# TangJiakai/RecBole-FairRec

Hardware: AMD Instinct MI355X
Metric: training interactions/sec + achieved HBM GB/s, FOCF emb=64 at 1/2/4/8 MI355X (higher is better)
Workload: dtype f32; 1 GPU; FOCF fair_objective=value, 1000001 users x 100001 items, embedding_size=64, B=8192 per GPU, Adam lr=1e-3 weight_decay=1e-3 (BASELINE.json configs[1]); ranks_seen=1, item_distribution=uniform, launch=hipGraph, lazy_adam_sweep_period=123, tables=single GPU, global_batch=8192, aged_steps=123

## Files before the change

### include/fairrec_hip.h

```cpp
#ifndef FAIRREC_HIP_H
#define FAIRREC_HIP_H

#include <stddef.h>
#include <stdint.h>

#ifdef __cplusplus
extern "C" {
#endif

#if defined(__GNUC__) || defined(__clang__)
#define FR_API __attribute__((visibility("default")))
#else
#define FR_API
#endif

#define FR_OK 0
#define FR_EINVAL (-1)
#define FR_EHIP (-2)
#define FR_EUNSUPPORTED (-3)

#define FR_DEV_ERR_INDEX_RANGE 1u
#define FR_DEV_ERR_SST_GROUPS 2u

#define FR_DEV_ERR_BUCKET_OVERFLOW 4u
// ... 57 lines not shown
    const float* sst;
    int64_t B;
    void* ws;
    size_t ws_bytes;
    const float* rating;
} fr_focf_batch;
FR_API int fr_focf_prepare_many(const fr_focf_batch* batches, int32_t n, int64_t n_users, int64_t n_items, int32_t dim,
                         uint32_t* err_flag, void* stream);

FR_API int fr_focf_clip_grad_norm(const fr_table* U, const fr_table* I, int64_t B, float max_norm,
                           const float* extra_sqnorm, float* norm_out, void* ws, size_t ws_bytes, void* stream);

FR_API int fr_focf_backward_adam(const fr_table* U, const fr_table* I, const fr_adam* adam, int64_t B,
                          int32_t sweep_period, void* ws, size_t ws_bytes, void* stream);

FR_API int fr_focf_prepare_step(const fr_focf_batch* batches, const int32_t* stamps, int32_t n, const fr_table* U,
                                const fr_table* I, int32_t replay_cap, uint32_t* err_flag, void* stream);
FR_API int fr_focf_step(const fr_table* U, const fr_table* I, const fr_adam* adam, const int64_t* user,
                        const int64_t* item, const float* rating, const float* sst, int64_t B, int32_t objective,
                        float fair_weight, int32_t sweep_period, int32_t stamp, void* ws, size_t ws_bytes,
                        float* loss_out, void* prev_ws, int64_t prev_B, float* prev_loss_out, float* loss_acc,
                        uint32_t* err_flag, void* stream);
FR_API int fr_focf_step_finish(void* ws, size_t ws_bytes, int64_t B, int32_t dim, int32_t objective, float fair_weight,
                               float* loss_out, float* loss_acc, void* stream);
FR_API int fr_focf_step_runs(const fr_table* U, const fr_table* I, const fr_adam* adam, const int64_t* user,
                             const int64_t* item, const float* rating, const float* sst, int64_t B, int32_t objective,
                             float fair_weight, int32_t sweep_period, int32_t stamp, void* ws, size_t ws_bytes, void* prev_ws,
                             int64_t prev_B, float* prev_loss_out, float* loss_acc, uint32_t* err_flag, void* stream);
FR_API int fr_focf_step_runs_pipe(const fr_table* U, const fr_table* I, const fr_adam* adam, const int64_t* user,
                                  const int64_t* item, const float* rating, const float* sst, int64_t B, int32_t objective,
                                  float fair_weight, int32_t sweep_period, int32_t stamp, void* ws, size_t ws_bytes, void* fin_ws,
                                  int64_t fin_B, int32_t fin_step, void* prev_ws, int64_t prev_B, float* prev_loss_out,
                                  float* loss_acc, int32_t* own_u, int32_t* own_i, uint32_t* err_flag, void* stream);

FR_API size_t fr_focf_row_words(int64_t n_users, int64_t n_items);
FR_API int fr_focf_stage(const fr_table* U, const fr_table* I, const fr_focf_batch* claim, int32_t claim_stamp,
                         int32_t claim_gen, const fr_focf_batch* place, int32_t place_stamp, int32_t place_gen,
                         int32_t sweep_period, uint64_t* row_words, uint32_t* err_flag, void* stream);
FR_API int fr_focf_step_staged(const fr_table* U, const fr_table* I, const fr_adam* adam, const float* sst, int64_t B,
                               int32_t objective, float fair_weight, int32_t sweep_period, int32_t stamp, int32_t gen,
                               void* ws, size_t ws_bytes, void* prev_ws, int64_t prev_B, float* prev_loss_out,
                               float* loss_acc, uint64_t* row_words, const fr_focf_batch* claim, int32_t claim_stamp,
                               int32_t claim_gen, const fr_focf_batch* place, int32_t place_stamp, int32_t place_gen,
                               uint32_t* err_flag, void* stream);
FR_API int fr_focf_step_finish_staged(void* ws, size_t ws_bytes, int64_t B, int32_t dim, int32_t objective,
                                      float fair_weight, float* loss_out, float* loss_acc, void* stream);
FR_API int fr_focf_runs_many(const fr_table* U, const fr_table* I, const fr_adam* adam, const fr_focf_batch* batches,
                             int32_t n, int32_t objective, float fair_weight, int32_t sweep_period, int32_t first_stamp,
                             void* fin_ws, int64_t fin_B, int32_t fin_step, float* fin_loss_out, void* prev_ws, int64_t prev_B,
                             float* prev_loss_out, float* loss_ring, int32_t loss_slots, int32_t first_slot, float* loss_acc,
                             int32_t* own_u, int32_t* own_i, uint32_t* err_flag, void* stream);
FR_API int fr_focf_steps_many(const fr_table* U, const fr_table* I, const fr_adam* adam, const fr_focf_batch* batches,
                              int32_t n, int32_t objective, float fair_weight, int32_t sweep_period, int32_t first_stamp,
                              int32_t first_gen, void* prev_ws, int64_t prev_B, float* prev_loss_out, float* loss_ring,
                              int32_t loss_slots, int32_t first_slot, float* loss_acc, uint64_t* row_words,
                              uint32_t* err_flag, void* stream);

FR_API int fr_focf_predict(const fr_table* U, const fr_table* I, const fr_adam* adam, const int64_t* user,
                    const int64_t* item, int64_t B, float max_rating, float* out, uint32_t* err_flag, void* stream);


FR_API int fr_table_flush(const fr_table* t, const fr_adam* adam, void* stream);

FR_API int fr_table_gather(const fr_table* t, const fr_adam* adam, const int64_t* idx, int64_t M, float* out,
                    uint32_t* err_flag, void* stream);

// ... 435 lines not shown
```

### recbole-fairrec_amd/csrc/focf_gather.hpp

```cpp
#pragma once
#include "common.hpp"
#include "kernels.hpp"
#include "table.hpp"
#include "focf_ws.hpp"

namespace fr {

template <int E, int NWAVES = GATHER_THREADS / WAVE>
struct GatherLds {
    float red[NWAVES];
    float irow[NWAVES][3][64 * E + 1];
};

struct SortedPark {
    const int32_t* pos_of;
    const int4* info;
    const float* sst;
    int4* recs;
    int4* vals;
    float* mse_e;
};

struct PipeWait {
    const int32_t *own_prev_u, *own_prev_i;
    int32_t *own_cur_u, *own_cur_i;
    int fin_step;
};

template <int E>
__device__ __forceinline__ int pipe_take_row(const TableV& T, int row, int need, RowFrag<E>& p, RowFrag<E>& m, RowFrag<E>& v,
                                             int lane, uint32_t* err) {
    int l = 0;
    for (int spin = 0; spin < (1 << 18); ++spin) {
        l = __hip_atomic_load(T.last + row, __ATOMIC_RELAXED, __HIP_MEMORY_SCOPE_AGENT);
        if (l >= need) break;
        __builtin_amdgcn_s_sleep(8);
    }
    l = uniform(l);
    if (l < need && lane == 0 && err) atomicOr(err, FR_DEV_ERR_PIPE_WAIT);
    const int D = T.D;
#pragma unroll
    for (int e = 0; e < E; ++e) {
        const int d = lane + 64 * e;
        const size_t o = (size_t)row * D + d;
        p.x[e] = d < D ? __hip_atomic_load(T.p + o, __ATOMIC_RELAXED, __HIP_MEMORY_SCOPE_AGENT) : 0.f;
        m.x[e] = d < D ? __hip_atomic_load(T.m + o, __ATOMIC_RELAXED, __HIP_MEMORY_SCOPE_AGENT) : 0.f;
        v.x[e] = d < D ? __hip_atomic_load(T.v + o, __ATOMIC_RELAXED, __HIP_MEMORY_SCOPE_AGENT) : 0.f;
    }
    return l;
}

template <int E, bool TRAIN, bool SHARE, bool SORTED = false, bool PIPE = false, int NW = GATHER_THREADS / WAVE>
__device__ __forceinline__ void focf_gather_body(
    const TableV& U, const TableV& I, const AdamC& c, const int64_t* __restrict__ user, const int64_t* __restrict__ item,
    const float* __restrict__ rating, int B, int upto_u, int upto_i, const FocfWs& w, float max_rating,
    float* __restrict__ predict_out, uint32_t* err, int block, GatherLds<SHARE ? E : 0, NW>& lds, SortedPark sp = SortedPark{},
    PipeWait pw = PipeWait{}) {
    static_assert(NW % 4 == 0, "squared errors are reduced four waves at a time");
    const int lane = threadIdx.x & 63;
    const int wib = threadIdx.x >> 6;
    const int b = block * NW + wib;
    const bool valid = b < B;
    const int D = U.D;
    float e2 = 0.f;
    int ur = 0, ir = -1 - wib;
    int js = b;
    int4 inf = make_int4(0, 0, 0, 0);
    float sv = 0.f;
    if (SORTED && valid) {
        js = sp.pos_of[b];
        inf = sp.info[b];
        if (sp.sst) sv = sp.sst[b];
    }
    if (valid) {
        long long ul = user[b], il = item[b];
        if (ul < 0 || ul >= U.n_rows || il < 0 || il >= I.n_rows) {
            if (lane == 0 && err) atomicOr(err, FR_DEV_ERR_INDEX_RANGE);
            ul = ul < 0 || ul >= U.n_rows ? 0 : ul;
            il = il < 0 || il >= I.n_rows ? 0 : il;
        }
        ur = uniform((int)ul);
        ir = uniform((int)il);
    }
    int lead = wib;
    bool shares = false;
    if (SHARE) {
        int it[NW];
#pragma unroll
        for (int q = 0; q < NW; ++q) {
            const int bq = block * NW + q;
            long long v = bq < B ? item[bq] : -1;
            it[q] = (v < 0 || v >= I.n_rows) ? (bq < B ? 0 : -1 - q) : (int)v;
        }
#pragma unroll
        for (int q = NW - 1; q >= 0; --q) {
            if (q < wib && it[q] == ir) lead = q;
#pragma unroll
            for (int r = 0; r < q; ++r) shares |= it[q] == it[r];
        }
    }
    lead = uniform(lead);
    shares = uniform((int)shares) != 0;
    RowFrag<E> pu, mu, vu, pi, mi, vi;
    if (valid) {
        int lu = U.last[ur];
        int li = lead == wib ? I.last[ir] : 0;
        int ou = -1, oi = -1;
        if (PIPE) {
            ou = pw.own_prev_u[ur];
            if (lead == wib) oi = pw.own_prev_i[ir];
        }
        load_row<E>(pu, U.p + (size_t)ur * D, D, lane);
        if (lead == wib) load_row<E>(pi, I.p + (size_t)ir * D, D, lane);
        load_row<E>(mu, U.m + (size_t)ur * D, D, lane);
        load_row<E>(vu, U.v + (size_t)ur * D, D, lane);
        if (lead == wib) {
            load_row<E>(mi, I.m + (size_t)ir * D, D, lane);
            load_row<E>(vi, I.v + (size_t)ir * D, D, lane);
        }
        if (PIPE) {
            if (pw.fin_step >= 0 && uniform(ou) == pw.fin_step) lu = pipe_take_row<E>(U, ur, pw.fin_step, pu, mu, vu, lane, err);
            if (lead == wib && pw.fin_step >= 0 && uniform(oi) == pw.fin_step)
                li = pipe_take_row<E>(I, ir, pw.fin_step, pi, mi, vi, lane, err);
            if (lane == 0) {
                pw.own_cur_u[ur] = upto_u + 1;
                if (lead == wib) pw.own_cur_i[ir] = upto_i + 1;
            }
        }
#ifdef FR_DIAG_GATHER_NO_REPLAY
        if (PIPE) lu = upto_u, li = upto_i;
#endif
        const int t0u = uniform(lu);
        if (lead != wib) {
            replay<E>(pu, mu, vu, t0u, upto_u, c, lane);
        } else {
            const int t0i = uniform(li);
            if (upto_u == upto_i) {
                if (t0u < t0i) replay<E>(pu, mu, vu, t0u, t0i, c, lane);
                else if (t0i < t0u) replay<E>(pi, mi, vi, t0i, t0u, c, lane);
                replay2<E>(pu, mu, vu, pi, mi, vi, t0u > t0i ? t0u : t0i, upto_u, c, lane);
            } else {
                replay<E>(pu, mu, vu, t0u, upto_u, c, lane);
                replay<E>(pi, mi, vi, t0i, upto_i, c, lane);
            }
        }
    }
    if (SHARE && shares) {
        if (valid && lead == wib) {
#pragma unroll
            for (int e = 0; e < E; ++e) {
                lds.irow[wib][0][lane + 64 * e] = pi.x[e];
                lds.irow[wib][1][lane + 64 * e] = mi.x[e];
// ... 260 lines not shown
```

### recbole-fairrec_amd/csrc/focf_runs.hip

```cpp
#include <stddef.h>
#include <stdlib.h>

#include <algorithm>
#include <vector>

#include "common.hpp"
#include "kernels.hpp"
#include "table.hpp"
#include "focf_ws.hpp"
#include "focf_loss.hpp"
#include "focf_gather.hpp"

namespace fr {

#ifndef FR_RUN_WAVES
#define FR_RUN_WAVES 8
#endif
constexpr int RUN_WAVES = FR_RUN_WAVES;
constexpr int RUN_THREADS = 64 * RUN_WAVES;
#ifndef FR_RUN_DIAG
#define FR_RUN_DIAG 0
#endif
#ifndef FR_RUN_MB1
#define FR_RUN_MB1 8
// ... 376 lines not shown
    blk -= 1;
    if (blk >= a.n_item_blocks) {
        const long long wave = (long long)(blk - a.n_item_blocks) * RUN_WAVES + wv;
        if (wave < a.n_sweep_waves) sweep_slice_wave<E>(a.U, a.I, a.c, a.sw, a.sweep_wave0 + wave, lane);
        return;
    }
    for (int k = blk; k < a.B; k += a.n_item_blocks) {
        const int rK = G(a.w.nseg_i)[0], rj0 = G(a.w.seg_start_i)[k], rj1 = G(a.w.seg_start_i)[k + 1];
        const int rir = G(a.w.seg_row_i)[k];
        if (k >= uniform(rK) || FR_RUN_DIAG == 4) break;
        const int j0 = uniform(rj0);
        run_finish_item<E>(a, k, j0, uniform(rj1) - j0, uniform(rir), lds_rows, coef_s, sh, lane, wv);
        __syncthreads();
    }
}

#ifndef FR_PIPE_MB
#define FR_PIPE_MB 4
#endif
struct PipeArgs {
    RunArgs fin;
    TableV U, I;
    AdamC c;
    const int64_t *user, *item;
    const float* rating;
    int B, upto;
    FocfWs w;
    SortedPark sp;
    PipeWait pw;
    uint32_t* err;
    int n_fin_blocks, n_gather_blocks, n_sweep_blocks, n_sweep_front;
    SweepSlice sw;
    long long n_sweep_waves;
};

#ifndef FR_PIPE_PRIO
#define FR_PIPE_PRIO 1
#endif
#ifndef FR_PIPE_WPE
#define FR_PIPE_WPE 8
#endif
#ifndef FR_PIPE_PAIR_MAX_E
#define FR_PIPE_PAIR_MAX_E 0
#endif
__host__ __device__ constexpr bool pipe_pair(int E) { return E <= FR_PIPE_PAIR_MAX_E; }
#ifdef FR_PIPE_TRACE
__device__ unsigned long long pipe_dbg[8 * 8];
struct PipeSpan {
    int role, slot;
    __device__ PipeSpan(int r, int step) : role(r), slot(step & 7) {
        if (r == 0 && threadIdx.x < 8) pipe_dbg[((step + 4) & 7) * 8 + threadIdx.x] = (threadIdx.x & 1) ? 0ull : ~0ull;
        if (threadIdx.x == 0 && (blockIdx.x & 15) == 0) atomicMin(&pipe_dbg[slot * 8 + 2 * role], __builtin_amdgcn_s_memrealtime());
    }
    __device__ ~PipeSpan() {
        if ((threadIdx.x & 63) == 0 && (blockIdx.x & 15) == 0) atomicMax(&pipe_dbg[slot * 8 + 2 * role + 1], __builtin_amdgcn_s_memrealtime());
    }
};
#define PIPE_SPAN(r) PipeSpan span_(r, p.upto)
#else
#define PIPE_SPAN(r) do {} while (0)
#endif

template <int E>
__global__ __launch_bounds__(RUN_THREADS) __attribute__((amdgpu_waves_per_eu(FR_PIPE_WPE, FR_PIPE_WPE))) void focf_runs_pipe_kernel(PipeArgs p) {
    constexpr int CAP = run_cap(E);
    __shared__ __align__(16) float lds_rows[CAP * 64 * E];
    __shared__ float coef_s[CAP];
    __shared__ float sh[4];
    using GLds = GatherLds<E, pipe_pair(E) ? 2 * RUN_WAVES : RUN_WAVES>;
    static_assert(sizeof(GLds) <= sizeof(lds_rows), "the gather's LDS fits the item runs' row buffer");
    GLds& glds = *reinterpret_cast<GLds*>(lds_rows);
    const int lane = threadIdx.x & 63, wv = threadIdx.x >> 6;
    int blk = (int)blockIdx.x;
    if (blk == 0) {
        PIPE_SPAN(0);
        const RunArgs a = args_through_vgprs<RunArgs>(lane);
        if (a.prev.loss_out && threadIdx.x < 256) step_reduce_loss<256>(a.prev);
        return;
    }
    blk -= 1;
    if (blk < p.n_sweep_front) {
        PIPE_SPAN(1);
        const long long wave = (long long)blk * RUN_WAVES + wv;
        if (wave < p.n_sweep_waves) sweep_slice_wave<E>(p.U, p.I, p.c, p.sw, wave, lane);
        return;
    }
    blk -= p.n_sweep_front;
    if (blk < p.n_fin_blocks) {
        PIPE_SPAN(2);
#if FR_PIPE_PRIO
        __builtin_amdgcn_s_setprio(3);
#endif
        const RunArgs a = args_through_vgprs<RunArgs>(lane);
        for (int k = blk; k < a.B; k += a.n_item_blocks) {
            const int rK = G(a.w.nseg_i)[0], rj0 = G(a.w.seg_start_i)[k], rj1 = G(a.w.seg_start_i)[k + 1];
            const int rir = G(a.w.seg_row_i)[k];
            if (k >= uniform(rK)) break;
            const int j0 = uniform(rj0);
            run_finish_item<E, FR_PIPE_MB>(a, k, j0, uniform(rj1) - j0, uniform(rir), lds_rows, coef_s, sh, lane, wv);
            __syncthreads();
        }
        return;
    }
    blk -= p.n_fin_blocks;
    if (blk < p.n_gather_blocks) {
        PIPE_SPAN(3);
#if FR_PIPE_PRIO
        __builtin_amdgcn_s_setprio(2);
#endif
        if (blk == 0 && threadIdx.x == 0) *p.w.defer = DeferLoss{nullptr, 0, 0.f, 0};
        if constexpr (pipe_pair(E))
            focf_gather_pair_body<E, RUN_WAVES>(p.U, p.I, p.c, p.user, p.item, p.rating, p.B, p.upto, p.w, p.err, blk, glds, p.sp, p.pw);
        else
            focf_gather_body<E, true, true, true, true, RUN_WAVES>(p.U, p.I, p.c, p.user, p.item, p.rating, p.B, p.upto, p.upto, p.w,
                                                                   0.f, nullptr, p.err, blk, glds, p.sp, p.pw);
        return;
    }
    blk -= p.n_gather_blocks;
    {
        PIPE_SPAN(1);
        const long long wave = (long long)(p.n_sweep_front + blk) * RUN_WAVES + wv;
        if (wave < p.n_sweep_waves) sweep_slice_wave<E>(p.U, p.I, p.c, p.sw, wave, lane);
    }
}

}

using namespace fr;

#ifdef FR_PIPE_TRACE
extern "C" __attribute__((visibility("default"))) int fr_debug_pipe_trace(unsigned long long* out, int reset) {
    if (hipMemcpyFromSymbol(out, HIP_SYMBOL(pipe_dbg), sizeof(unsigned long long) * 64) != hipSuccess) return -1;
    if (reset) {
        unsigned long long init[64];
        for (int i = 0; i < 64; ++i) init[i] = (i & 1) ? 0ull : ~0ull;
        if (hipMemcpyToSymbol(HIP_SYMBOL(pipe_dbg), init, sizeof(init)) != hipSuccess) return -1;
    }
    return 0;
}
#endif

extern "C" int fr_focf_step_runs_pipe(const fr_table* U, const fr_table* I, const fr_adam* adam, const int64_t* user,
                                      const int64_t* item, const float* rating, const float* sst, int64_t B, int32_t objective,
                                      float fair_weight, int32_t sweep_period, int32_t stamp, void* ws, size_t ws_bytes,
                                      void* fin_ws, int64_t fin_B, int32_t fin_step, void* prev_ws, int64_t prev_B,
                                      float* prev_loss_out, float* loss_acc, int32_t* own_u, int32_t* own_i, uint32_t* err_flag,
                                      void* stream_) {
    hipStream_t stream = (hipStream_t)stream_;
    int rc;
    if ((rc = check_table(U, "fr_focf_step_runs_pipe(U)")) || (rc = check_table(I, "fr_focf_step_runs_pipe(I)")) ||
        (rc = check_focf_adam(adam, "fr_focf_step_runs_pipe")))
        return rc;
    const bool gather = user != nullptr && B > 0, finish = fin_ws != nullptr && fin_B > 0;
    FR_CHECK_ARG(U->dim == I->dim && U->step >= 1 && U->step == I->step && !U->step_dev && !I->step_dev,
                 "fr_focf_step_runs_pipe: tables of one width at one host-side step");
    FR_CHECK_ARG(objective >= FR_FOCF_NONE && objective <= FR_FOCF_OVER, "fr_focf_step_runs_pipe: objective %d", objective);
    FR_CHECK_ARG(!gather || (item && rating && ws && own_u && own_i && B <= FR_SORT_MAX && (objective == FR_FOCF_NONE || sst)),
                 "fr_focf_step_runs_pipe: bad batch");
    FR_CHECK_ARG(!finish || (fin_step >= 1 && fin_B <= FR_SORT_MAX && (!gather || fin_step == U->step - 1)),
                 "fr_focf_step_runs_pipe: the batch to finish must be the previous step's");
    PipeArgs p{};
    p.c = make_adamc(adam);
    p.err = err_flag;
    RunArgs& a = p.fin;
    a.c = p.c;
    a.objective = objective;
    a.fair_weight = fair_weight;
    a.err = err_flag;
    a.publish = gather ? 1 : 0;
    fr_table Uf = *U, If = *I;
    if (finish) {
        Uf.step = If.step = fin_step;
        a.w = focf_layout(fin_ws, fin_B, U->dim);
        a.B = (int)fin_B;
        a.n_item_blocks = (int)std::min<long long>(FR_RUN_ITEM_BLOCKS, fin_B);
    }
    a.U = view(&Uf);
    a.I = view(&If);
    a.prev = prev_of(prev_ws, prev_B, U->dim, objective, fair_weight, prev_loss_out, loss_acc, false);
    p.n_fin_blocks = a.n_item_blocks;
    if (gather) {
        p.w = focf_layout(ws, B, U->dim);
        FR_CHECK_ARG(ws_bytes >= p.w.bytes, "fr_focf_step_runs_pipe: workspace %zu < %zu bytes", ws_bytes, p.w.bytes);
        p.U = view(U);
        p.I = view(I);
        p.user = user;
        p.item = item;
        p.rating = rating;
        p.B = (int)B;
        p.upto = U->step - 1;
        p.sp = SortedPark{p.w.pos_i, p.w.info, sst, p.w.task_rec, p.w.task_info, p.w.mse_e};
        const int cur = U->step & 1, prv = cur ^ 1;
        p.pw = PipeWait{own_u + (size_t)prv * U->n_rows, own_i + (size_t)prv * I->n_rows, own_u + (size_t)cur * U->n_rows,
                        own_i + (size_t)cur * I->n_rows, finish ? fin_step : -1};
        const int per_block = pipe_pair((U->dim + 63) / 64) ? 2 * RUN_WAVES : RUN_WAVES;
        p.n_gather_blocks = (int)((B + per_block - 1) / per_block);
        if (sweep_period > 0) {
            p.sw = make_sweep_slice(U, I, sweep_period);
            p.sw.skip_from = finish ? std::min(stamp, fin_step) : stamp;
            p.n_sweep_waves = sweep_slice_waves(p.sw);
        }
    }
    p.n_sweep_blocks = (int)((p.n_sweep_waves + RUN_WAVES - 1) / RUN_WAVES);
    static const int front_pct = getenv("FAIRREC_PIPE_SWEEP_FRONT") ? atoi(getenv("FAIRREC_PIPE_SWEEP_FRONT")) : 100;
    p.n_sweep_front = (int)((long long)p.n_sweep_blocks * std::min(std::max(front_pct, 0), 100) / 100);
    const long long blocks = 1 + p.n_sweep_blocks + p.n_fin_blocks + p.n_gather_blocks;
    ProfScope prof(K_FOCF_STEP, stream);
    FR_DISPATCH_E(U->dim, FR_LAUNCH(prof, (focf_runs_pipe_kernel<E>), dim3((unsigned)blocks), dim3(RUN_THREADS), 0, stream, p));
    FR_CHECK_LAUNCH();
    return FR_OK;
}

extern "C" int fr_focf_step_runs(const fr_table* U, const fr_table* I, const fr_adam* adam, const int64_t* user,
                                 const int64_t* item, const float* rating, const float* sst, int64_t B, int32_t objective,
                                 float fair_weight, int32_t sweep_period, int32_t stamp, void* ws, size_t ws_bytes, void* prev_ws,
                                 int64_t prev_B, float* prev_loss_out, float* loss_acc, uint32_t* err_flag, void* stream_) {
    hipStream_t stream = (hipStream_t)stream_;
    int rc;
    if ((rc = check_table(U, "fr_focf_step_runs(U)")) || (rc = check_table(I, "fr_focf_step_runs(I)")) ||
        (rc = check_focf_adam(adam, "fr_focf_step_runs")))
        return rc;
    FR_CHECK_ARG(U->dim == I->dim, "fr_focf_step_runs: user dim %d != item dim %d", U->dim, I->dim);
    FR_CHECK_ARG(ws && user && item && rating, "fr_focf_step_runs: null pointer");
    FR_CHECK_ARG(objective >= FR_FOCF_NONE && objective <= FR_FOCF_OVER,
                 "fr_focf_step_runs: objective %d needs batch-wide statistics before the update (use fr_focf_forward)", objective);
    FR_CHECK_ARG(objective == FR_FOCF_NONE || sst, "fr_focf_step_runs: sst column required for a fairness objective");
    FR_CHECK_ARG(B >= 1 && B <= FR_SORT_MAX, "fr_focf_step_runs: batch size %lld not in 1..%d", (long long)B, FR_SORT_MAX);
    FR_CHECK_ARG(U->step >= 1 && U->step == I->step, "fr_focf_step_runs: table.step must be the step being applied (>=1), "
                 "the same for both tables");
    FR_CHECK_ARG(!U->step_dev && !I->step_dev, "fr_focf_step_runs: device step counters are not supported");
    RunArgs a{};
    a.w = focf_layout(ws, B, U->dim);
    FR_CHECK_ARG(ws_bytes >= a.w.bytes, "fr_focf_step_runs: workspace %zu < %zu bytes", ws_bytes, a.w.bytes);
    a.U = view(U);
    a.I = view(I);
    a.c = make_adamc(adam);
    a.B = (int)B;
    a.objective = objective;
    a.fair_weight = fair_weight;
    a.err = err_flag;
    static const int split_pct = getenv("FAIRREC_RUNS_SWEEP_SPLIT") ? atoi(getenv("FAIRREC_RUNS_SWEEP_SPLIT")) : 0;
    long long sweep_blocks = 0, in_gather = 0;
    if (sweep_period > 0) {
// ... 50 lines not shown
            if (done[1]) (void)hipEventDestroy(done[1]);
        }
    } ev;
    if (ss && n > G) {
        FR_CHECK_HIP(hipEventCreateWithFlags(&ev.fork, hipEventDisableTiming));
        FR_CHECK_HIP(hipEventCreateWithFlags(&ev.done[0], hipEventDisableTiming));
        FR_CHECK_HIP(hipEventCreateWithFlags(&ev.done[1], hipEventDisableTiming));
    }
    hipEvent_t ev_fork = ev.fork;
    hipEvent_t* ev_done = ev.done;
    int rc;
    auto prepare = [&](int g, hipStream_t st) {
        const int lo = g * G, cnt = std::min(G, n - lo);
        return fr_focf_prepare_step(batches + lo, stamps.data() + lo, cnt, U, I, sweep_period, err_flag, st);
    };
    if ((rc = prepare(0, stream))) return rc;
    fr_table tu = *U, ti = *I;
    for (int k = 0; k < n; ++k) {
        if (k % G == 0) {
            const int g = k / G;
            if (g > 0 && ss) FR_CHECK_HIP(hipStreamWaitEvent(stream, ev_done[g & 1], 0));
            if ((g + 1) * G < n) {
                if (ss) {
                    FR_CHECK_HIP(hipEventRecord(ev_fork, stream));
                    FR_CHECK_HIP(hipStreamWaitEvent(ss->stream, ev_fork, 0));
                    if ((rc = prepare(g + 1, ss->stream))) return rc;
                    FR_CHECK_HIP(hipEventRecord(ev_done[(g + 1) & 1], ss->stream));
                } else if ((rc = prepare(g + 1, stream))) {
                    return rc;
                }
            }
        }
        const fr_focf_batch& b = batches[k];
        rc = fr_focf_step_runs_pipe(&tu, &ti, adam, b.user, b.item, b.rating, b.sst, b.B, objective, fair_weight, sweep_period,
                                    stamps[(size_t)k], b.ws, b.ws_bytes, fin_ws, fin_B, fin_step, prev_ws, prev_B, prev_loss_out,
                                    loss_acc, own_u, own_i, err_flag, stream_);
        if (rc) return rc;
        prev_ws = fin_ws; prev_B = fin_B; prev_loss_out = fin_loss_out;
        fin_ws = b.ws; fin_B = b.B; fin_step = tu.step;
        fin_loss_out = loss_ring + 4 * (size_t)((first_slot + k) % loss_slots);
        ++tu.step; ++ti.step;
    }
    return FR_OK;
}
```

### recbole-fairrec_amd/fairrec/_C.py

```python
from __future__ import annotations

import ctypes
import os
from ctypes import POINTER, Structure, c_char_p, c_double, c_float, c_int, c_int32, c_int64, c_size_t, c_uint32, c_uint64, c_void_p

LIB_PATH = os.environ.get("FAIRREC_HIP_LIB") or os.path.join(os.path.dirname(os.path.abspath(__file__)), "lib",
                                                             "libfairrec_hip.so")

FR_SORT_MAX = 16384
DEV_ERR_INDEX_RANGE = 1
DEV_ERR_SST_GROUPS = 2
DEV_ERR_BUCKET_OVERFLOW = 4
DEV_ERR_PIPE_WAIT = 8
DEV_ERR_SAMPLE_ROUNDS = 16
EUNSUPPORTED = -3
WGRAD_MAX = 8
FR_TOPK_MAX = 256
MLP_INFER_MAX_LAYERS = 8
MLP_INFER_MAX_WIDTH = 512
MLP_INFER_MAX_NETS = 8
PAIR_MLP_MAX_LINEARS = 6
PAIR_MLP_MAX_WIDTH = 256

FOCF_OBJECTIVES = {"none": 0, "value": 1, "absolute": 2, "under": 3, "over": 4, "nonparity": 5}
# ... 67 lines not shown


class FairrecError(RuntimeError):
    pass


_PROTOS = {
    "fr_version": (c_int, []),
    "fr_last_error": (c_char_p, []),
    "fr_sort_segments": (c_int, [c_void_p, c_int64, c_int64, c_void_p, c_void_p, c_void_p, c_void_p, c_void_p,
                                 c_void_p, c_void_p]),
    "fr_focf_workspace_bytes": (c_size_t, [c_int64, c_int32]),
    "fr_focf_forward": (c_int, [POINTER(FrTable), POINTER(FrTable), POINTER(FrAdam), c_void_p, c_void_p, c_void_p,
                                c_void_p, c_int64, c_int32, c_float, c_int32, c_void_p, c_size_t, c_void_p, c_void_p,
                                c_void_p, c_void_p]),
    "fr_focf_prepare": (c_int, [c_void_p, c_void_p, c_void_p, c_int64, c_int64, c_int64, c_int32, c_void_p, c_size_t,
                                c_void_p, c_void_p]),
    "fr_focf_prepare_many": (c_int, [POINTER(FrFocfBatch), c_int32, c_int64, c_int64, c_int32, c_void_p, c_void_p]),
    "fr_focf_clip_grad_norm": (c_int, [POINTER(FrTable), POINTER(FrTable), c_int64, c_float, c_void_p, c_void_p,
                                       c_void_p, c_size_t, c_void_p]),
    "fr_focf_backward_adam": (c_int, [POINTER(FrTable), POINTER(FrTable), POINTER(FrAdam), c_int64, c_int32,
                                      c_void_p, c_size_t, c_void_p]),
    "fr_focf_prepare_step": (c_int, [POINTER(FrFocfBatch), POINTER(c_int32), c_int32, POINTER(FrTable), POINTER(FrTable),
                                     c_int32, c_void_p, c_void_p]),
    "fr_focf_step": (c_int, [POINTER(FrTable), POINTER(FrTable), POINTER(FrAdam), c_void_p, c_void_p, c_void_p, c_void_p,
                             c_int64, c_int32, c_float, c_int32, c_int32, c_void_p, c_size_t, c_void_p, c_void_p, c_int64,
                             c_void_p, c_void_p, c_void_p, c_void_p]),
    "fr_focf_step_runs": (c_int, [POINTER(FrTable), POINTER(FrTable), POINTER(FrAdam), c_void_p, c_void_p, c_void_p, c_void_p,
                                  c_int64, c_int32, c_float, c_int32, c_int32, c_void_p, c_size_t, c_void_p, c_int64, c_void_p,
                                  c_void_p, c_void_p, c_void_p]),
    "fr_focf_step_runs_pipe": (c_int, [POINTER(FrTable), POINTER(FrTable), POINTER(FrAdam), c_void_p, c_void_p, c_void_p, c_void_p,
                                       c_int64, c_int32, c_float, c_int32, c_int32, c_void_p, c_size_t, c_void_p, c_int64, c_int32,
                                       c_void_p, c_int64, c_void_p, c_void_p, c_void_p, c_void_p, c_void_p, c_void_p]),
    "fr_focf_step_finish": (c_int, [c_void_p, c_size_t, c_int64, c_int32, c_int32, c_float, c_void_p, c_void_p,
                                    c_void_p]),
    "fr_side_stream_handle": (c_void_p, []),
    "fr_focf_row_words": (c_size_t, [c_int64, c_int64]),
    "fr_focf_stage": (c_int, [POINTER(FrTable), POINTER(FrTable), POINTER(FrFocfBatch), c_int32, c_int32,
                              POINTER(FrFocfBatch), c_int32, c_int32, c_int32, c_void_p, c_void_p, c_void_p]),
    "fr_focf_step_staged": (c_int, [POINTER(FrTable), POINTER(FrTable), POINTER(FrAdam), c_void_p, c_int64, c_int32, c_float,
                                    c_int32, c_int32, c_int32, c_void_p, c_size_t, c_void_p, c_int64, c_void_p, c_void_p,
                                    c_void_p, POINTER(FrFocfBatch), c_int32, c_int32, POINTER(FrFocfBatch), c_int32, c_int32,
                                    c_void_p, c_void_p]),
    "fr_focf_step_finish_staged": (c_int, [c_void_p, c_size_t, c_int64, c_int32, c_int32, c_float, c_void_p, c_void_p,
                                           c_void_p]),
    "fr_focf_compose_epoch": (c_int, [c_void_p, c_void_p, c_int64, c_void_p, c_int64, c_int64, c_int64, c_void_p, c_int64,
                                      c_void_p, c_int64, c_void_p]),
    "fr_randperm_workspace_bytes": (c_size_t, [c_int64]),
    "fr_randperm": (c_int, [c_void_p, c_int64, c_void_p, c_void_p, c_size_t, c_void_p]),
    "fr_focf_runs_many": (c_int, [POINTER(FrTable), POINTER(FrTable), POINTER(FrAdam), c_void_p, c_int32, c_int32, c_float,
                                  c_int32, c_int32, c_void_p, c_int64, c_int32, c_void_p, c_void_p, c_int64, c_void_p, c_void_p,
                                  c_int32, c_int32, c_void_p, c_void_p, c_void_p, c_void_p, c_void_p]),
    "fr_focf_steps_many": (c_int, [POINTER(FrTable), POINTER(FrTable), POINTER(FrAdam), c_void_p, c_int32, c_int32, c_float,
                                   c_int32, c_int32, c_int32, c_void_p, c_int64, c_void_p, c_void_p, c_int32, c_int32, c_void_p,
                                   c_void_p, c_void_p, c_void_p]),
    "fr_focf_predict": (c_int, [POINTER(FrTable), POINTER(FrTable), POINTER(FrAdam), c_void_p, c_void_p, c_int64,
                                c_float, c_void_p, c_void_p, c_void_p]),
    "fr_table_flush": (c_int, [POINTER(FrTable), POINTER(FrAdam), c_void_p]),
    "fr_table_gather": (c_int, [POINTER(FrTable), POINTER(FrAdam), c_void_p, c_int64, c_void_p, c_void_p,
                                c_void_p]),
    "fr_table_train_workspace_bytes": (c_size_t, [c_int64, c_int32]),
    "fr_table_segments_bytes": (c_size_t, [c_int64]),
    "fr_table_gather_train": (c_int, [POINTER(FrTable), POINTER(FrAdam), c_void_p, c_int64, c_int32, c_int32, c_void_p,
                                      c_void_p, c_size_t, c_void_p, c_void_p]),
    "fr_table_gather_train_prepared": (c_int, [POINTER(FrTable), POINTER(FrAdam), c_void_p, c_int64, c_int32, c_int32,
                                               c_void_p, c_void_p, c_size_t, c_void_p, c_void_p]),
# ... 308 lines not shown
```

### recbole-fairrec_amd/fairrec/model/fair_recommender/focf.py

```python
from __future__ import annotations

import ctypes
import math
import os
from typing import Dict, Optional

import torch
import torch.nn as nn

from ... import _C
from ...optim import AdamHyper, FusedLazyAdam, LazyTable
from ...utils.enum_type import InputType
from ..abstract_recommender import FairRecommender
from ..init import xavier_normal_initialization


_BATCH_DTYPE = [("user", "<u8"), ("item", "<u8"), ("sst", "<u8"), ("B", "<i8"), ("ws", "<u8"), ("ws_bytes", "<u8"),
                ("rating", "<u8")]


class _LossHandle(torch.autograd.Function):

    @staticmethod
    def forward(ctx, loss, engine, *weights):
# ... 18 lines not shown
    PIPE = os.environ.get("FAIRREC_FOCF_PIPE", "1") == "1"

    def __init__(self, user_weight: torch.Tensor, item_weight: torch.Tensor, objective: str, fair_weight: float,
                 max_rating: float):
        if user_weight.device.type != "cuda":
            raise _C.FairrecError("FOCF runs only on a ROCm device (model.to('cuda')); there is no CPU fallback")
        _C.lib()
        self.device = user_weight.device
        self.U = LazyTable(user_weight)
        self.I = LazyTable(item_weight)
        self.objective = _C.FOCF_OBJECTIVES[objective]
        self.fair_weight = float(fair_weight)
        self.max_rating = float(max_rating)
        self.hyper = AdamHyper(device=self.device, cap=1)
        self.optimizer: Optional[FusedLazyAdam] = None
        self.sweep_period: Optional[int] = None
        self.ws = [None] * self.N_WS
        self.ws_cur = 0
        self._side = None
        self._prep = {}
        self.loss_ring = torch.zeros((self.LOSS_SLOTS, 4), dtype=torch.float32, device=self.device)
        self._loss_views = [self.loss_ring[k] for k in range(self.LOSS_SLOTS)]
        self._ws_need = {}
        self.loss_slot = 0
        self.err_flag = torch.zeros(1, dtype=torch.int32, device=self.device)
        self.pending_B = 0
        self.backward_seen = False
        self.defer_loss = False
        self.item_runs = False
        self.fused_step = True
        self._stash = None
        self._prev = None
        self._pipe = None
        self._own = None
        self._stamp_last = 0
        self._stamp_gen = (self.U.stamp_gen, self.I.stamp_gen)
        self.loss_acc = torch.zeros(8, dtype=torch.float32, device=self.device)
        self.staged = self.STAGED
        self._st = {}
        self._row_words = None
        self._ws_dirty = set()
        self._gen_cur = None

    def tables(self) -> Dict[str, LazyTable]:
        if self._pipe is not None:
            self.finish()
        return {"user_embedding_layer.weight": self.U, "item_embedding_layer.weight": self.I}

    def bind_optimizer(self, opt: FusedLazyAdam, sweep_period: Optional[int]):
        self.optimizer = opt
        self.hyper = opt.hyper
        self.sweep_period = sweep_period
        for t in (self.U, self.I):
            t.ensure_state()

    def _sweep(self, B: int) -> int:
        if self.sweep_period is not None:
            return int(self.sweep_period)
        return max(8, math.ceil(max(self.U.n_rows, self.I.n_rows) / max(B, 1)))

    def _workspace(self, B: int, k: int):
        need = self._ws_need.get(B)
        if need is None:
            need = self._ws_need[B] = _C.lib().fr_focf_workspace_bytes(B, self.U.dim)
        if self.ws[k] is None or self.ws[k].numel() < need:
            self.ws[k] = torch.zeros(need, dtype=torch.uint8, device=self.device)
# ... 196 lines not shown
        stamp = None
        if hit is not None:
            self.ws_cur, group, stamp = hit
            if not group["joined"]:
                torch.cuda.current_stream().wait_event(group["done"])
                group["joined"] = True
            flags = 1
        else:
            held = [t[0] for t in (self._prev, self._pipe) if t is not None]
            taken = {v[0] for v in self._prep.values()}
            while any(w is self.ws[self.ws_cur] for w in held) or (held and self.ws_cur in taken):
                self.ws_cur = (self.ws_cur + 1) % self.N_WS
        if self.defer_loss and self.optimizer is not None:
            flags |= 2
        if self.item_runs:
            flags |= 4
        ws = self._workspace(B, self.ws_cur)
        coming = []
        if next_batch is not None:
            coming = [next_batch] if isinstance(next_batch[0], torch.Tensor) else [nb for nb in next_batch if nb is not None]
        if self._prep and (hit is None or len(self._prep) > len(coming)):
            alive = {self._key(nb[0], nb[1]) for nb in coming}
            for k in [k for k in self._prep if k not in alive]:
                torch.cuda.current_stream().wait_event(self._prep.pop(k)[1]["done"])
        fused = (self.fused_step and self.defer_loss and self.optimizer is not None and self.objective != 5 and not want_pred
                 and (not self.item_runs or (self.RUNS and rating is not None)) and self.U.step == self.I.step)
        if self._pipe is not None and not (fused and self.item_runs and self.PIPE):
            self.finish()
        stamp_now = self._next_stamp() if (fused and stamp is None) else None
        if coming and len(self._prep) <= self.LOW_WATER:
            todo = [nb for nb in coming if self._key(nb[0], nb[1]) not in self._prep]
            if todo:
                self.prepare_many(todo[:self.GROUP], ahead=1)
        self.loss_slot = (self.loss_slot + 1) % self.LOSS_SLOTS
        loss = self._loss_views[self.loss_slot]
        self.hyper.check_step(self.U.step + 1)
        if fused:
            if stamp is None:
                arr = (_C.FrFocfBatch * 1)(_C.FrFocfBatch(user.data_ptr(), item.data_ptr(),
                                                          _C.ptr(sst if self.objective != 0 else None), B, ws.data_ptr(),
                                                          ws.numel(), rating.data_ptr()))
                stamp = stamp_now
                tu, ti = self.U.c(), self.I.c()
                rc = _C.lib().fr_focf_prepare_step(arr, (ctypes.c_int32 * 1)(stamp), 1, ctypes.byref(tu), ctypes.byref(ti),
                                                   self._sweep(B), self.err_flag.data_ptr(), _C.current_stream())
                _C.check(rc, "fr_focf_prepare_step")
            self._stash = (user, item, rating, sst, B, ws, stamp, loss)
            self._stash_runs = bool(self.item_runs)
            self.pending_B = B
            return loss, None
        pred = torch.empty(B, dtype=torch.float32, device=self.device) if want_pred else None
        return self._forward_chain(user, item, rating, sst, B, flags, ws, loss, pred)

    def _forward_chain(self, user, item, rating, sst, B, flags, ws, loss, pred):
        tu, ti = self.U.c(self.U.step + 1), self.I.c(self.I.step + 1)
        rc = _C.lib().fr_focf_forward(ctypes.byref(tu), ctypes.byref(ti), ctypes.byref(self.hyper.c()),
                                      user.data_ptr(), item.data_ptr(), rating.data_ptr(), _C.ptr(sst), B,
                                      self.objective, self.fair_weight, flags, ws.data_ptr(), ws.numel(),
                                      loss.data_ptr(), _C.ptr(pred), self.err_flag.data_ptr(), _C.current_stream())
        _C.check(rc, "fr_focf_forward")
        self.pending_B = B
        return loss, pred

    def clip_grad_norm(self, max_norm: float, group=None):
        if self.pending_B == 0:
            raise _C.FairrecError("clip_grad_norm without a preceding calculate_loss()")
# ... 22 lines not shown
            raise _C.FairrecError("no optimizer bound: build fairrec.optim.FusedLazyAdam(model.hip_engine(), ...)")
        B = self.pending_B
        tu, ti = self.U.c(self.U.step + 1), self.I.c(self.I.step + 1)
        if self._stash is not None and len(self._stash) > 8:
            user, item, rating, sst, B, ws, stamp, loss, claim, place = self._stash
            self._stash = None
            if self._prev is not None and not self._prev[3]:
                self.finish()
            pw, pB, ploss, _ = self._prev if self._prev is not None else (None, 0, None, True)
            rc = _C.lib().fr_focf_step_staged(ctypes.byref(tu), ctypes.byref(ti), ctypes.byref(self.hyper.c()), _C.ptr(sst), B,
                                              self.objective, self.fair_weight, self._sweep(B), stamp[0], stamp[1],
                                              ws.data_ptr(), ws.numel(), _C.ptr(pw), pB, _C.ptr(ploss),
                                              self.loss_acc.data_ptr(), self._words().data_ptr(),
                                              ctypes.byref(claim["batch"]) if claim else None, claim["stamp"] if claim else 0,
                                              claim["gen"] if claim else 0,
                                              ctypes.byref(place["batch"]) if place else None, place["stamp"] if place else 0,
                                              place["gen"] if place else 0, self.err_flag.data_ptr(), _C.current_stream())
            _C.check(rc, "fr_focf_step_staged")
            if claim:
                claim["stage"] = 1
            if place:
                place["stage"] = 2
            self._prev = (ws, B, loss, True)
            self._keep = (user, item, rating, sst)
        elif self._stash is not None:
            user, item, rating, sst, B, ws, stamp, loss = self._stash
            self._stash = None
            if self._prev is not None and self._prev[3]:
                self.finish()
            pw, pB, ploss, _ = self._prev if self._prev is not None else (None, 0, None, False)
            if getattr(self, "_stash_runs", False) and self.PIPE:
                fin = self._pipe
                own_u, own_i = self._own_arrays()
                rc = _C.lib().fr_focf_step_runs_pipe(ctypes.byref(tu), ctypes.byref(ti), ctypes.byref(self.hyper.c()),
                                                     user.data_ptr(), item.data_ptr(), rating.data_ptr(), _C.ptr(sst), B,
                                                     self.objective, self.fair_weight, self._sweep(B), stamp, ws.data_ptr(),
                                                     ws.numel(), _C.ptr(fin[0]) if fin else None, fin[1] if fin else 0,
                                                     fin[2] if fin else 0, _C.ptr(pw), pB, _C.ptr(ploss), self.loss_acc.data_ptr(),
                                                     own_u.data_ptr(), own_i.data_ptr(), self.err_flag.data_ptr(),
                                                     _C.current_stream())
                _C.check(rc, "fr_focf_step_runs_pipe")
                self._pipe = (ws, B, self.U.step + 1, loss, (user, item, rating, sst))
                self._prev = (fin[0], fin[1], fin[3], False) if fin else None
                self._keep = (user, item, rating, sst)
                self.U.step += 1
                self.I.step += 1
                self.U._dirty = self.I._dirty = True
                self.pending_B = 0
                self.backward_seen = False
                return
            if self._pipe is not None:
                self.finish()
                pw, pB, ploss, _ = self._prev if self._prev is not None else (None, 0, None, False)
            if getattr(self, "_stash_runs", False):
                rc = _C.lib().fr_focf_step_runs(ctypes.byref(tu), ctypes.byref(ti), ctypes.byref(self.hyper.c()),
                                                user.data_ptr(), item.data_ptr(), rating.data_ptr(), _C.ptr(sst), B,
                                                self.objective, self.fair_weight, self._sweep(B), stamp, ws.data_ptr(),
                                                ws.numel(), _C.ptr(pw), pB, _C.ptr(ploss), self.loss_acc.data_ptr(),
                                                self.err_flag.data_ptr(), _C.current_stream())
                _C.check(rc, "fr_focf_step_runs")
            else:
                rc = _C.lib().fr_focf_step(ctypes.byref(tu), ctypes.byref(ti), ctypes.byref(self.hyper.c()),
                                           user.data_ptr(), item.data_ptr(), rating.data_ptr(), _C.ptr(sst), B,
                                           self.objective, self.fair_weight, self._sweep(B), stamp, ws.data_ptr(), ws.numel(),
                                           loss.data_ptr(), _C.ptr(pw), pB, _C.ptr(ploss), self.loss_acc.data_ptr(),
                                           self.err_flag.data_ptr(), _C.current_stream())
                _C.check(rc, "fr_focf_step")
            self._prev = (ws, B, loss, False)
            self._keep = (user, item, rating, sst)
        else:
            rc = _C.lib().fr_focf_backward_adam(ctypes.byref(tu), ctypes.byref(ti), ctypes.byref(self.hyper.c()), B,
                                                self._sweep(B), self.ws[self.ws_cur].data_ptr(),
                                                self.ws[self.ws_cur].numel(), _C.current_stream())
            _C.check(rc, "fr_focf_backward_adam")
# ... 340 lines not shown
```

Measured before the change: 289.9 million interactions/s.

## Pre-catch-up next batch's item rows inside pipe kernel and add fresh gather fast path

Adds catch-up blocks to the pipelined FOCF step kernel. These replay lazy Adam updates on the next batch's item rows ahead of time, provided those rows are not held by the current or finishing batch. In the gather, the per-wave item loads are replaced by a lane readlane broadcast. A 'fresh' fast path skips the cross-step pipe waits and item replay when every item row in the block is already up to date, writing side buffers directly. The goal is to take item replay and pipe-wait latency off the gather's critical path, at the cost of extra catch-up blocks, redundant row loads and more complex staleness logic.

```diff
diff --git a/include/fairrec_hip.h b/include/fairrec_hip.h
--- a/include/fairrec_hip.h
+++ b/include/fairrec_hip.h
@@ -113,6 +113,12 @@
                                   float fair_weight, int32_t sweep_period, int32_t stamp, void* ws, size_t ws_bytes, void* fin_ws,
                                   int64_t fin_B, int32_t fin_step, void* prev_ws, int64_t prev_B, float* prev_loss_out,
                                   float* loss_acc, int32_t* own_u, int32_t* own_i, uint32_t* err_flag, void* stream);
+FR_API int fr_focf_step_runs_pipe_next(const fr_table* U, const fr_table* I, const fr_adam* adam, const int64_t* user,
+                                       const int64_t* item, const float* rating, const float* sst, int64_t B, int32_t objective,
+                                       float fair_weight, int32_t sweep_period, int32_t stamp, void* ws, size_t ws_bytes,
+                                       void* fin_ws, int64_t fin_B, int32_t fin_step, void* prev_ws, int64_t prev_B,
+                                       float* prev_loss_out, float* loss_acc, int32_t* own_u, int32_t* own_i, uint32_t* err_flag,
+                                       void* next_ws, int64_t next_B, void* stream);
 
 FR_API size_t fr_focf_row_words(int64_t n_users, int64_t n_items);
 FR_API int fr_focf_stage(const fr_table* U, const fr_table* I, const fr_focf_batch* claim, int32_t claim_stamp,
diff --git a/recbole-fairrec_amd/csrc/focf_gather.hpp b/recbole-fairrec_amd/csrc/focf_gather.hpp
--- a/recbole-fairrec_amd/csrc/focf_gather.hpp
+++ b/recbole-fairrec_amd/csrc/focf_gather.hpp
@@ -26,6 +26,10 @@
     int32_t *own_cur_u, *own_cur_i;
     int fin_step;
 };
+
+#ifdef FR_PIPE_TRACE
+static __device__ unsigned long long pipe_dbg_fresh[2];
+#endif
 
 template <int E>
 __device__ __forceinline__ int pipe_take_row(const TableV& T, int row, int need, RowFrag<E>& p, RowFrag<E>& m, RowFrag<E>& v,
@@ -67,6 +71,14 @@
     int js = b;
     int4 inf = make_int4(0, 0, 0, 0);
     float sv = 0.f;
+    int itl = -1 - (lane & (NW - 1));
+    if (SHARE) {
+        const int bq = block * NW + (lane & (NW - 1));
+        if (bq < B) {
+            const long long v = item[bq];
+            itl = (v < 0 || v >= I.n_rows) ? 0 : (int)v;
+        }
+    }
     if (SORTED && valid) {
         js = sp.pos_of[b];
         inf = sp.info[b];
@@ -84,14 +96,15 @@
     }
     int lead = wib;
     bool shares = false;
+#ifdef FR_DIAG_GATHER_NO_FRESH
+    constexpr bool FRESH = false;
+#else
+    constexpr bool FRESH = PIPE && SORTED && SHARE;
+#endif
     if (SHARE) {
         int it[NW];
 #pragma unroll
-        for (int q = 0; q < NW; ++q) {
-            const int bq = block * NW + q;
-            long long v = bq < B ? item[bq] : -1;
-            it[q] = (v < 0 || v >= I.n_rows) ? (bq < B ? 0 : -1 - q) : (int)v;
-        }
+        for (int q = 0; q < NW; ++q) it[q] = __builtin_amdgcn_readlane(itl, q);
 #pragma unroll
         for (int q = NW - 1; q >= 0; --q) {
             if (q < wib && it[q] == ir) lead = q;
@@ -102,22 +115,75 @@
     lead = uniform(lead);
     shares = uniform((int)shares) != 0;
     RowFrag<E> pu, mu, vu, pi, mi, vi;
+    const bool first = FRESH && valid && js == (inf.z & 0xffff);
+    int lu = 0, li = 0, ou = -1, oi = -1;
+    int ll = upto_i, ol = -1;
+    if (FRESH && itl >= 0) {
+        ll = I.last[itl];
+        if (pw.fin_step >= 0) ol = pw.own_prev_i[itl];
+    }
     if (valid) {
-        int lu = U.last[ur];
-        int li = lead == wib ? I.last[ir] : 0;
-        int ou = -1, oi = -1;
+        lu = U.last[ur];
+        li = lead == wib ? I.last[ir] : 0;
         if (PIPE) {
             ou = pw.own_prev_u[ur];
             if (lead == wib) oi = pw.own_prev_i[ir];
         }
         load_row<E>(pu, U.p + (size_t)ur * D, D, lane);
-        if (lead == wib) load_row<E>(pi, I.p + (size_t)ir * D, D, lane);
+        if (FRESH || lead == wib) load_row<E>(pi, I.p + (size_t)ir * D, D, lane);
         load_row<E>(mu, U.m + (size_t)ur * D, D, lane);
         load_row<E>(vu, U.v + (size_t)ur * D, D, lane);
-        if (lead == wib) {
+        if (lead == wib || first) {
             load_row<E>(mi, I.m + (size_t)ir * D, D, lane);
             load_row<E>(vi, I.v + (size_t)ir * D, D, lane);
         }
+    }
+    bool fresh = false;
+    if (FRESH) {
+        const bool stale = itl >= 0 && (ll != upto_i || (pw.fin_step >= 0 && ol == pw.fin_step));
+        fresh = __ballot(stale) == 0ull;
+#ifdef FR_PIPE_TRACE
+        if (threadIdx.x == 0) atomicAdd(&pipe_dbg_fresh[fresh ? 0 : 1], 1ull);
+#endif
+    }
+    if (FRESH && fresh) {
+        if (valid) {
+            if (pw.fin_step >= 0 && uniform(ou) == pw.fin_step) lu = pipe_take_row<E>(U, ur, pw.fin_step, pu, mu, vu, lane, err);
+            if (lane == 0) {
+                pw.own_cur_u[ur] = upto_u + 1;
+                if (lead == wib) pw.own_cur_i[ir] = upto_i + 1;
+            }
+#ifdef FR_DIAG_GATHER_NO_REPLAY
+            lu = upto_u;
+#endif
+            replay<E>(pu, mu, vu, uniform(lu), upto_u, c, lane);
+            float dot = 0.f;
+#pragma unroll
+            for (int e = 0; e < E; ++e) dot = fmaf(pu.x[e], pi.x[e], dot);
+            dot = wave_sum(dot);
+            const size_t so = (size_t)uniform(js) * D;
+            store_row<E>(pu, w.side[0] + so, D, lane);
+            store_row<E>(mu, w.side[1] + so, D, lane);
+            store_row<E>(vu, w.side[2] + so, D, lane);
+            store_row<E>(pi, w.side[3] + so, D, lane);
+            if (first) {
+                store_row<E>(mi, w.side[4] + so, D, lane);
+                store_row<E>(vi, w.side[5] + so, D, lane);
+            }
+            const float er = dot - rating[b];
+            if (lane == 0) {
+                atomicMax(&U.stamp[ur], upto_u + 1);
+                atomicMax(&I.stamp[ir], upto_i + 1);
+                const float cm = 2.f * er / (float)B;
+                sp.recs[js] = make_int4(ur, inf.x, inf.y, b);
+                sp.vals[js] = make_int4(__float_as_int(rating[b]), __float_as_int(sv), __float_as_int(dot), __float_as_int(cm));
+                sp.mse_e[b] = er * er;
+            }
+        }
+        if (block == 0 && threadIdx.x == 0) *w.ticket = 0u;
+        return;
+    }
+    if (valid) {
         if (PIPE) {
             if (pw.fin_step >= 0 && uniform(ou) == pw.fin_step) lu = pipe_take_row<E>(U, ur, pw.fin_step, pu, mu, vu, lane, err);
             if (lead == wib && pw.fin_step >= 0 && uniform(oi) == pw.fin_step)
diff --git a/recbole-fairrec_amd/csrc/focf_runs.hip b/recbole-fairrec_amd/csrc/focf_runs.hip
--- a/recbole-fairrec_amd/csrc/focf_runs.hip
+++ b/recbole-fairrec_amd/csrc/focf_runs.hip
@@ -432,7 +432,45 @@
     int n_fin_blocks, n_gather_blocks, n_sweep_blocks, n_sweep_front;
     SweepSlice sw;
     long long n_sweep_waves;
+    const int32_t *nx_nseg, *nx_rows, *cu_nseg, *cu_rows, *fi_nseg, *fi_rows;
+    int nx_B, n_catch_blocks;
+    int catch_upto, catch_skip_from;
 };
+
+#ifndef FR_PIPE_CATCH_BLOCKS
+#define FR_PIPE_CATCH_BLOCKS 16
+#endif
+#ifndef FR_PIPE_CATCH_MAX_ITEMS
+#define FR_PIPE_CATCH_MAX_ITEMS 512
+#endif
+
+template <int E>
+__device__ __forceinline__ void pipe_catch_up_items(const PipeArgs& p, int task, int n_tasks, int lane) {
+    const int Kn = uniform(G(p.nx_nseg)[0]), Kc = uniform(G(p.cu_nseg)[0]);
+    const int Kf = p.fi_nseg ? uniform(G(p.fi_nseg)[0]) : 0;
+    if (Kn > FR_PIPE_CATCH_MAX_ITEMS || Kc > FR_PIPE_CATCH_MAX_ITEMS || Kf > FR_PIPE_CATCH_MAX_ITEMS) return;
+    const int D = p.I.D, upto = p.catch_upto;
+    for (int j = task; j < Kn && j < p.nx_B; j += n_tasks) {
+        const int row = uniform(G(p.nx_rows)[j]);
+        if (row < 0 || row >= p.I.n_rows) continue;
+        bool held = false;
+        for (int q = lane; q < Kc && q < p.B; q += 64) held |= G(p.cu_rows)[q] == row;
+        for (int q = lane; q < Kf && q < p.fin.B; q += 64) held |= G(p.fi_rows)[q] == row;
+        const int st = p.I.stamp[row], lt = p.I.last[row];
+        RowFrag<E> pr, mr, vr;
+        load_row<E>(pr, p.I.p + (size_t)row * D, D, lane);
+        load_row<E>(mr, p.I.m + (size_t)row * D, D, lane);
+        load_row<E>(vr, p.I.v + (size_t)row * D, D, lane);
+        if (__ballot(held) != 0ull || uniform(st) < p.catch_skip_from) continue;
+        const int t0 = uniform(lt);
+        if (t0 >= upto) continue;
+        replay<E>(pr, mr, vr, t0, upto, p.c, lane);
+        store_row<E>(pr, p.I.p + (size_t)row * D, D, lane);
+        store_row<E>(mr, p.I.m + (size_t)row * D, D, lane);
+        store_row<E>(vr, p.I.v + (size_t)row * D, D, lane);
+        if (lane == 0) p.I.last[row] = upto;
+    }
+}
 
 #ifndef FR_PIPE_PRIO
 #define FR_PIPE_PRIO 1
@@ -479,6 +517,12 @@
         return;
     }
     blk -= 1;
+    if (blk < p.n_catch_blocks) {
+        PIPE_SPAN(1);
+        pipe_catch_up_items<E>(p, blk * RUN_WAVES + wv, p.n_catch_blocks * RUN_WAVES, lane);
+        return;
+    }
+    blk -= p.n_catch_blocks;
     if (blk < p.n_sweep_front) {
         PIPE_SPAN(1);
         const long long wave = (long long)blk * RUN_WAVES + wv;
@@ -538,14 +582,17 @@
     }
     return 0;
 }
-#endif
-
-extern "C" int fr_focf_step_runs_pipe(const fr_table* U, const fr_table* I, const fr_adam* adam, const int64_t* user,
-                                      const int64_t* item, const float* rating, const float* sst, int64_t B, int32_t objective,
-                                      float fair_weight, int32_t sweep_period, int32_t stamp, void* ws, size_t ws_bytes,
-                                      void* fin_ws, int64_t fin_B, int32_t fin_step, void* prev_ws, int64_t prev_B,
-                                      float* prev_loss_out, float* loss_acc, int32_t* own_u, int32_t* own_i, uint32_t* err_flag,
-                                      void* stream_) {
+extern "C" __attribute__((visibility("default"))) int fr_debug_pipe_fresh(unsigned long long* out) {
+    return hipMemcpyFromSymbol(out, HIP_SYMBOL(pipe_dbg_fresh), sizeof(unsigned long long) * 2) == hipSuccess ? 0 : -1;
+}
+#endif
+
+static int focf_step_runs_pipe_impl(const fr_table* U, const fr_table* I, const fr_adam* adam, const int64_t* user,
+                                    const int64_t* item, const float* rating, const float* sst, int64_t B, int32_t objective,
+                                    float fair_weight, int32_t sweep_period, int32_t stamp, void* ws, size_t ws_bytes,
+                                    void* fin_ws, int64_t fin_B, int32_t fin_step, void* prev_ws, int64_t prev_B,
+                                    float* prev_loss_out, float* loss_acc, int32_t* own_u, int32_t* own_i, uint32_t* err_flag,
+                                    void* next_ws, int64_t next_B, void* stream_) {
     hipStream_t stream = (hipStream_t)stream_;
     int rc;
     if ((rc = check_table(U, "fr_focf_step_runs_pipe(U)")) || (rc = check_table(I, "fr_focf_step_runs_pipe(I)")) ||
@@ -600,15 +647,53 @@
             p.sw.skip_from = finish ? std::min(stamp, fin_step) : stamp;
             p.n_sweep_waves = sweep_slice_waves(p.sw);
         }
+        static const bool catch_on = !(getenv("FAIRREC_PIPE_CATCH_UP") && atoi(getenv("FAIRREC_PIPE_CATCH_UP")) == 0);
+        if (next_ws && next_B > 0 && next_B <= FR_SORT_MAX && next_ws != ws && next_ws != fin_ws && catch_on) {
+            const FocfWs nx = focf_layout(next_ws, next_B, U->dim);
+            p.nx_nseg = nx.nseg_i;
+            p.nx_rows = nx.seg_row_i;
+            p.nx_B = (int)next_B;
+            p.cu_nseg = p.w.nseg_i;
+            p.cu_rows = p.w.seg_row_i;
+            if (finish) {
+                p.fi_nseg = a.w.nseg_i;
+                p.fi_rows = a.w.seg_row_i;
+            }
+            p.catch_upto = U->step;
+            p.catch_skip_from = finish ? std::min(stamp, fin_step) : stamp;
+            p.n_catch_blocks = (int)std::min<long long>(FR_PIPE_CATCH_BLOCKS, (std::min<long long>(next_B, FR_PIPE_CATCH_MAX_ITEMS) + RUN_WAVES - 1) / RUN_WAVES);
+        }
     }
     p.n_sweep_blocks = (int)((p.n_sweep_waves + RUN_WAVES - 1) / RUN_WAVES);
     static const int front_pct = getenv("FAIRREC_PIPE_SWEEP_FRONT") ? atoi(getenv("FAIRREC_PIPE_SWEEP_FRONT")) : 100;
     p.n_sweep_front = (int)((long long)p.n_sweep_blocks * std::min(std::max(front_pct, 0), 100) / 100);
-    const long long blocks = 1 + p.n_sweep_blocks + p.n_fin_blocks + p.n_gather_blocks;
+    const long long blocks = 1 + p.n_catch_blocks + p.n_sweep_blocks + p.n_fin_blocks + p.n_gather_blocks;
     ProfScope prof(K_FOCF_STEP, stream);
     FR_DISPATCH_E(U->dim, FR_LAUNCH(prof, (focf_runs_pipe_kernel<E>), dim3((unsigned)blocks), dim3(RUN_THREADS), 0, stream, p));
     FR_CHECK_LAUNCH();
     return FR_OK;
+}
+
+extern "C" int fr_focf_step_runs_pipe(const fr_table* U, const fr_table* I, const fr_adam* adam, const int64_t* user,
+                                      const int64_t* item, const float* rating, const float* sst, int64_t B, int32_t objective,
+                                      float fair_weight, int32_t sweep_period, int32_t stamp, void* ws, size_t ws_bytes,
+                                      void* fin_ws, int64_t fin_B, int32_t fin_step, void* prev_ws, int64_t prev_B,
+                                      float* prev_loss_out, float* loss_acc, int32_t* own_u, int32_t* own_i, uint32_t* err_flag,
+                                      void* stream_) {
+    return focf_step_runs_pipe_impl(U, I, adam, user, item, rating, sst, B, objective, fair_weight, sweep_period, stamp, ws, ws_bytes,
+                                    fin_ws, fin_B, fin_step, prev_ws, prev_B, prev_loss_out, loss_acc, own_u, own_i, err_flag,
+                                    nullptr, 0, stream_);
+}
+
+extern "C" int fr_focf_step_runs_pipe_next(const fr_table* U, const fr_table* I, const fr_adam* adam, const int64_t* user,
+                                           const int64_t* item, const float* rating, const float* sst, int64_t B,
+                                           int32_t objective, float fair_weight, int32_t sweep_period, int32_t stamp, void* ws,
+                                           size_t ws_bytes, void* fin_ws, int64_t fin_B, int32_t fin_step, void* prev_ws,
+                                           int64_t prev_B, float* prev_loss_out, float* loss_acc, int32_t* own_u, int32_t* own_i,
+                                           uint32_t* err_flag, void* next_ws, int64_t next_B, void* stream_) {
+    return focf_step_runs_pipe_impl(U, I, adam, user, item, rating, sst, B, objective, fair_weight, sweep_period, stamp, ws, ws_bytes,
+                                    fin_ws, fin_B, fin_step, prev_ws, prev_B, prev_loss_out, loss_acc, own_u, own_i, err_flag,
+                                    next_ws, next_B, stream_);
 }
 
 extern "C" int fr_focf_step_runs(const fr_table* U, const fr_table* I, const fr_adam* adam, const int64_t* user,
@@ -725,9 +810,11 @@
             }
         }
         const fr_focf_batch& b = batches[k];
-        rc = fr_focf_step_runs_pipe(&tu, &ti, adam, b.user, b.item, b.rating, b.sst, b.B, objective, fair_weight, sweep_period,
-                                    stamps[(size_t)k], b.ws, b.ws_bytes, fin_ws, fin_B, fin_step, prev_ws, prev_B, prev_loss_out,
-                                    loss_acc, own_u, own_i, err_flag, stream_);
+        const bool next_ready = k + 1 < n && ((k + 1) % G != 0 || !ss);
+        rc = focf_step_runs_pipe_impl(&tu, &ti, adam, b.user, b.item, b.rating, b.sst, b.B, objective, fair_weight, sweep_period,
+                                      stamps[(size_t)k], b.ws, b.ws_bytes, fin_ws, fin_B, fin_step, prev_ws, prev_B,
+                                      prev_loss_out, loss_acc, own_u, own_i, err_flag, next_ready ? batches[k + 1].ws : nullptr,
+                                      next_ready ? batches[k + 1].B : 0, stream_);
         if (rc) return rc;
         prev_ws = fin_ws; prev_B = fin_B; prev_loss_out = fin_loss_out;
         fin_ws = b.ws; fin_B = b.B; fin_step = tu.step;
diff --git a/recbole-fairrec_amd/fairrec/_C.py b/recbole-fairrec_amd/fairrec/_C.py
--- a/recbole-fairrec_amd/fairrec/_C.py
+++ b/recbole-fairrec_amd/fairrec/_C.py
@@ -123,6 +123,10 @@
     "fr_focf_step_runs_pipe": (c_int, [POINTER(FrTable), POINTER(FrTable), POINTER(FrAdam), c_void_p, c_void_p, c_void_p, c_void_p,
                                        c_int64, c_int32, c_float, c_int32, c_int32, c_void_p, c_size_t, c_void_p, c_int64, c_int32,
                                        c_void_p, c_int64, c_void_p, c_void_p, c_void_p, c_void_p, c_void_p, c_void_p]),
+    "fr_focf_step_runs_pipe_next": (c_int, [POINTER(FrTable), POINTER(FrTable), POINTER(FrAdam), c_void_p, c_void_p, c_void_p,
+                                            c_void_p, c_int64, c_int32, c_float, c_int32, c_int32, c_void_p, c_size_t, c_void_p,
+                                            c_int64, c_int32, c_void_p, c_int64, c_void_p, c_void_p, c_void_p, c_void_p, c_void_p,
+                                            c_void_p, c_int64, c_void_p]),
     "fr_focf_step_finish": (c_int, [c_void_p, c_size_t, c_int64, c_int32, c_int32, c_float, c_void_p, c_void_p,
                                     c_void_p]),
     "fr_side_stream_handle": (c_void_p, []),
diff --git a/recbole-fairrec_amd/fairrec/model/fair_recommender/focf.py b/recbole-fairrec_amd/fairrec/model/fair_recommender/focf.py
--- a/recbole-fairrec_amd/fairrec/model/fair_recommender/focf.py
+++ b/recbole-fairrec_amd/fairrec/model/fair_recommender/focf.py
@@ -74,6 +74,7 @@
         self._stash = None
         self._prev = None
         self._pipe = None
+        self._next_ws = None
         self._own = None
         self._stamp_last = 0
         self._stamp_gen = (self.U.stamp_gen, self.I.stamp_gen)
@@ -336,6 +337,11 @@
             todo = [nb for nb in coming if self._key(nb[0], nb[1]) not in self._prep]
             if todo:
                 self.prepare_many(todo[:self.GROUP], ahead=1)
+        self._next_ws = None
+        if coming:
+            nxt = self._prep.get(self._key(coming[0][0], coming[0][1]))
+            if nxt is not None and nxt[1]["joined"] and nxt[2] is not None:
+                self._next_ws = (self.ws[nxt[0]], coming[0][0].numel())
         self.loss_slot = (self.loss_slot + 1) % self.LOSS_SLOTS
         loss = self._loss_views[self.loss_slot]
         self.hyper.check_step(self.U.step + 1)
@@ -424,14 +430,16 @@
             if getattr(self, "_stash_runs", False) and self.PIPE:
                 fin = self._pipe
                 own_u, own_i = self._own_arrays()
-                rc = _C.lib().fr_focf_step_runs_pipe(ctypes.byref(tu), ctypes.byref(ti), ctypes.byref(self.hyper.c()),
-                                                     user.data_ptr(), item.data_ptr(), rating.data_ptr(), _C.ptr(sst), B,
-                                                     self.objective, self.fair_weight, self._sweep(B), stamp, ws.data_ptr(),
-                                                     ws.numel(), _C.ptr(fin[0]) if fin else None, fin[1] if fin else 0,
-                                                     fin[2] if fin else 0, _C.ptr(pw), pB, _C.ptr(ploss), self.loss_acc.data_ptr(),
-                                                     own_u.data_ptr(), own_i.data_ptr(), self.err_flag.data_ptr(),
-                                                     _C.current_stream())
-                _C.check(rc, "fr_focf_step_runs_pipe")
+                nxt, self._next_ws = self._next_ws, None
+                rc = _C.lib().fr_focf_step_runs_pipe_next(ctypes.byref(tu), ctypes.byref(ti), ctypes.byref(self.hyper.c()),
+                                                          user.data_ptr(), item.data_ptr(), rating.data_ptr(), _C.ptr(sst), B,
+                                                          self.objective, self.fair_weight, self._sweep(B), stamp, ws.data_ptr(),
+                                                          ws.numel(), _C.ptr(fin[0]) if fin else None, fin[1] if fin else 0,
+                                                          fin[2] if fin else 0, _C.ptr(pw), pB, _C.ptr(ploss),
+                                                          self.loss_acc.data_ptr(), own_u.data_ptr(), own_i.data_ptr(),
+                                                          self.err_flag.data_ptr(), nxt[0].data_ptr() if nxt else None,
+                                                          nxt[1] if nxt else 0, _C.current_stream())
+                _C.check(rc, "fr_focf_step_runs_pipe_next")
                 self._pipe = (ws, B, self.U.step + 1, loss, (user, item, rating, sst))
                 self._prev = (fin[0], fin[1], fin[3], False) if fin else None
                 self._keep = (user, item, rating, sst)
```

Measured after the change: 289.2 million interactions/s. About the same (-0.2%).
